# bridgedp/hunter_bipedal_control

Measured on AMD Instinct MI355X. Metric: MPC+WBC updates/sec (batch=4096, N=100, 12-DoF), higher is better.
Workload: dtype f64; 1 GPU; 4096 distinct hunter instances (4096/GPU, state seed 1234 + id), trot gait from t = 0.1, cmd_vel (0.3, 0, 0, 0), N=100 shooting intervals (dt 0.015 s), node tables generated on the device (hb_refgen_update, per-knot IK joint references), 1 SQP iteration + WeightedWbc per update, x0 of every call perturbed by measurement noise (sigma 0.01) so that no call re-solves a converged problem: every line s; batch_per_gpu=4096, total_instances=4096, horizon_nodes=100

## Files before the change

hunter_bipedal_control_amd/csrc/hb_lq.hpp:

```cpp
#pragma once
#include "hb_model.hpp"
#include "hb_tile.hpp"

namespace hb {

struct DevConfig {
  double Q_diag[HB_NX];
  double R_FF_diag[12];
  double R_jj[HB_NJ * HB_NJ];
  double friction_mu, friction_reg, friction_gripper, friction_shift, fb_mu, fb_delta;
  double soft_w;
  double pos_b[2], vel_b[2], force_b[2], force_lim[2];
  double kp_normal, zv_gain, zv_off, xy_gain;
  double g_max, g_min, alpha_decay, alpha_min, gamma_c, armijo, delta_tol;
  double torque_limits[5];
  double wbc_mu, swing_kp, swing_kd, bh_kp, bh_kd, ba_kp, ba_kd, w_swing, w_base, w_force, wbc_eps;
  int wbc_max_iter, wbc_type;
  double default_joint_state[HB_NJ];
  int debug_stop;
  int wbc_reg_steps;
  int wbc_eps_mode;
};

constexpr int NU_T = 12;
constexpr int REC_LD = 36, REC_CV = 22, REC_CU = 23;
constexpr int REC_AB = 0;
constexpr int REC_PR = 792;
constexpr int REC_QT = 1224;
constexpr int REC_QT_PACKED = 254;
constexpr int REC_qT = REC_QT + REC_QT_PACKED;
HB_HD constexpr int rec_Qidx(int i, int c) { return (i * (43 - i)) / 2 + c; }
constexpr int REC_RICCATI_END = 1730;
constexpr int REC_KX = 1730;
constexpr int REC_KE = 1950;
constexpr int REC_Z = 1960;
constexpr int REC_DF = 2020;
constexpr int REC_QF = 2032;
constexpr int REC_RF = 2054;
constexpr int REC_META = 2076;
constexpr int REC_DT = REC_META + 6;
constexpr int REC_DQ = REC_META + 8;
constexpr int REC_RX_END = REC_DQ + 10;
constexpr int REC_SIZE = 2112;
constexpr int GAIN_SIZE = 288;
HB_HD constexpr int rec_A(int i, int c) { return REC_AB + i * REC_LD + c; }
HB_HD constexpr int rec_B(int i, int a) { return REC_AB + i * REC_LD + REC_CU + a; }
HB_HD constexpr int rec_b(int i) { return REC_AB + i * REC_LD + REC_CV; }
HB_HD constexpr int rec_P(int a, int c) { return REC_PR + a * REC_LD + c; }
HB_HD constexpr int rec_R(int a, int c) { return REC_PR + a * REC_LD + REC_CU + c; }
HB_HD constexpr int rec_r(int a) { return REC_PR + a * REC_LD + REC_CV; }
inline void rec_unpack(const double* rec, double* A, double* B, double* b, double* Q, double* P, double* R, double* q, double* r, int* n_til) {
  for (int i = 0; i < 22; ++i) {
    for (int c = 0; c < 22; ++c) {
      if (A) A[i * 22 + c] = rec[rec_A(i, c)];
      if (Q) Q[i * 22 + c] = rec[REC_QT + (i <= c ? rec_Qidx(i, c) : rec_Qidx(c, i))];
    }
    for (int a = 0; a < NU_T; ++a)
      if (B) B[i * NU_T + a] = rec[rec_B(i, a)];
    if (b) b[i] = rec[rec_b(i)];
    if (q) q[i] = rec[REC_qT + i];
  }
  for (int a = 0; a < NU_T; ++a) {
    for (int c = 0; c < 22; ++c)
      if (P) P[a * 22 + c] = rec[rec_P(a, c)];
    for (int c = 0; c < NU_T; ++c)
      if (R) R[a * NU_T + c] = rec[rec_R(a, c)];
    if (r) r[a] = rec[rec_r(a)];
  }
  if (n_til) *n_til = int(rec[REC_META]) + int(rec[REC_META + 1]);
}
HB_HD void rec_unpack_recovery(const double* rec, double* Kx, double* ke, double* Z, double* dF, double* qf, double* rf, double* meta,
                               double* dt, double* dq) {
  const auto copy = [rec](double* dst, int at, int n) {
    if (dst)
      for (int i = 0; i < n; ++i) dst[i] = rec[at + i];
  };
  copy(Kx, REC_KX, 220); copy(ke, REC_KE, 10); copy(Z, REC_Z, 60); copy(dF, REC_DF, 12); copy(qf, REC_QF, 22); copy(rf, REC_RF, 22);
  copy(meta, REC_META, 6); copy(dt, REC_DT, 1); copy(dq, REC_DQ, 10);
}

struct RelaxedBarrierD {
  double mu, delta;
  HB_HD double value(double h) const {
    if (h > delta) return -mu * log_t(h);
    const double z = (h - 2.0 * delta) * rcp_t(delta);
    return mu * (-log_t(delta) + 0.5 * z * z - 0.5);
  }
  HB_HD double d1(double h) const { const double r = rcp_t(h > delta ? h : delta); return h > delta ? -mu * r : mu * (h - 2.0 * delta) * r * r; }
  HB_HD double d2(double h) const { const double r = rcp_t(h > delta ? h : delta); return mu * r * r; }
};

struct LqLds {
  static constexpr int CDt = 0;
  static constexpr int rowval = CDt + 384;
  static constexpr int xs = rowval + 12;
  static constexpr int us = xs + 22;
  static constexpr int fv = us + 22;
  static constexpr int scal = fv;
  static constexpr int xe = fv + 24;
  static constexpr int xplus = xe;
  static constexpr int ABt = xe + 22;
  static constexpr int W = ABt + 528;
  static constexpr int Pj = W;
  static constexpr int LDK = 29;
  static constexpr int Kx = W + 230;
  static constexpr int Z = Kx + 23;
  static constexpr int GtG = Kx + 124;
  static constexpr int btmp = fv;
  static constexpr int ints = Kx + 10 * LDK;
  static constexpr int park = ints + 16;
  static constexpr int xnext_park = fv;
  static constexpr int tail_end = park + 22;
  static constexpr int Mm = ABt;
  static constexpr int RFF = Mm + 10 * LDK;
  static constexpr int qx = RFF + 36;
  static constexpr int ru = qx + 22;
  static constexpr int Qd = ru + 22;
  static constexpr int Rjj = Qd + 22;
  static constexpr int LJ = ABt;
#if defined(__HIP_DEVICE_COMPILE__)
  static constexpr int J1 = ABt + 528;
#else
  static constexpr int J1 = LJ + 4 * LEGJ_SIZE;
#endif
  static constexpr int J2 = J1 + 29 * 9;
  static constexpr int LVP = 27;
  static constexpr int LV = J2 + 29 * 9;
#if defined(__HIP_DEVICE_COMPILE__)
  static constexpr int p1_end = LV + 2 * LVP;
  static constexpr int SC = fv + 12;
  HB_HD static constexpr int fr_slot(int pt, int i) { return LV + pt * LVP + 15 + 6 * (i & 1) + 3 * (i >> 1); }
#else
  static constexpr int FRh = LV + 2 * LVP;
  static constexpr int SC = FRh + 24;
  static constexpr int p1_end = SC + 12;
  HB_HD static constexpr int fr_slot(int pt, int i) { return FRh + 12 * pt + 3 * i; }
#endif
  static constexpr int total = p1_end > tail_end ? p1_end : tail_end;
};
static_assert(LqLds::J1 >= LqLds::ABt + 528, "ABt is written while J1 / J2 are still being read");
static_assert(LqLds::park >= LqLds::J1, "the parked states are written behind the compose: they lie over J1 / J2 / the leg values, which it has finished with by then");
static_assert(LqLds::Rjj + 100 <= LqLds::ABt + 528, "M | R_FF | q_x | r_u | Q-diagonal | R_jj must fit over ABt");
#if defined(__HIP_DEVICE_COMPILE__)
static_assert(LqLds::total * 8 <= 12800, "k_lq: LDS per node must allow 12 workgroups per CU (10 allocation granules of 1280 B, DESIGN.md 3.1)");
#endif
HB_HD int cd_row(int dir) { return dir < 22 ? dir : dir - 12; }
HB_HD int j_row(int dir) { return dir < 6 ? dir : (dir < 22 ? dir - 3 : dir - 15); }
HB_HD int j_dir(int row) { return row < 6 ? row : (row < 19 ? row + 3 : row + 15); }
HB_HD int j_col(int frow) { return frow < 6 ? frow - 3 : (frow < 9 ? frow : frow - 6); }
HB_HD int j_frow(int col) { return col < 3 ? col + 3 : (col < 6 ? col + 6 : col); }
HB_HD int c_slot(int i, int a) { return a == 0 ? 8 + i : 4 * (i & 1) + 2 * (i >> 1) + (a - 1); }
HB_HD int slot_foot(int s) { return s < 8 ? (s >> 2) + 2 * ((s >> 1) & 1) : s - 8; }
HB_HD bool slot_normal(int s) { return s >= 8; }
HB_HD bool slot_is_eq(int s, int cfm) { return slot_normal(s) || ((cfm >> slot_foot(s)) & 1); }
HB_HD bool slot_is_soft(int s, int cfm) { return !slot_normal(s) && !((cfm >> slot_foot(s)) & 1); }
struct EqStepLive { int cfm; HB_HD bool operator()(int j) const { return j == 2 || ((cfm >> j) & 5) != 0; } };
struct SoftStepLive { int cfm; HB_HD bool operator()(int j) const { return j != 2 && ((~cfm >> j) & 5) != 0; } };

HB_HD LegLayout lq_leg_layout() { LegLayout l; l.compact = true; l.pair_sum = true; return l; }

struct NodeIn {
  const double* x;
  const double* u;
  const double* xnext;
  const double* xref;
  const double* swing;
  double dt;
  int mode;
  bool preloaded = false;
  double x_lane = 0.0, u_lane = 0.0;
  const LegJointConst* jc = nullptr;
  bool consts = false;
  double c_tab = 0.0;
};

struct LqP1 {
  double *xs, *us, *xe, *fv, *LV_all, *SC, *J1, *J2, *CDt, *rowval, *LJ_all;
};
HB_HD LqP1 lq_p1(double* lds) {
  LqP1 p;
  p.xs = lds + LqLds::xs;
  p.us = lds + LqLds::us;
  p.xe = lds + LqLds::xe;
  p.fv = lds + LqLds::fv;
  p.LV_all = lds + LqLds::LV;
  p.SC = lds + LqLds::SC;
  p.J1 = lds + LqLds::J1;
  p.J2 = lds + LqLds::J2;
  p.CDt = lds + LqLds::CDt;
  p.rowval = lds + LqLds::rowval;
  p.LJ_all = lds + LqLds::LJ;
  return p;
}

HB_HD int lq_ms_slot(int pt, int e) { return (2 * pt + e / 5) * LEGJ_SIZE + (e % 5) * LEGJ_STRIDE + LEGJ_MS; }
constexpr int LQ_CV_IINV = 0, LQ_CV_WB = 6, LQ_CV_LJ = 9, LQ_CV_P = 12;
struct LqPointValues {
  Vec3<double> fr[HB_NC], fvel[HB_NC];
  Mat3<double> R;
  Vec3<double> wb, P, hb, lj, omega, euler_rate, v_lin, com_rel;
  Sym3<double> Iinv;
  double icy;
};
HB_HD void lq_point_values(const DevModel& M, const double* LV, const double* zyx_sc , const double* hn, LqPointValues& o) {
  const double mb = M.mass[0], mt = M.total_mass;
  const Vec3<double> cb(M.com[0][0], M.com[0][1], M.com[0][2]);
  Sym3<double> Ib;
  Ib.xx = M.inertia[0][0]; Ib.xy = M.inertia[0][1]; Ib.xz = M.inertia[0][2];
  Ib.yy = M.inertia[0][3]; Ib.yz = M.inertia[0][4]; Ib.zz = M.inertia[0][5];
  const Vec3<double> mc = ld3(LV + 0) + mb * cb;
  const Sym3<double> IO = ld6(LV + 3) + Ib + point_inertia<double>(mb, cb);
  o.lj = ld3(LV + 9);
  const Vec3<double> LjO = ld3(LV + 12);
  const double inv_m = rcp_t(mt);
  o.P = inv_m * mc;
  Sym3<double> Ic = IO;
  {
    const Sym3<double> sh = point_inertia<double>(mt, o.P);
    Ic.xx -= sh.xx; Ic.xy -= sh.xy; Ic.xz -= sh.xz; Ic.yy -= sh.yy; Ic.yz -= sh.yz; Ic.zz -= sh.zz;
  }
  {
    const double c00 = Ic.yy * Ic.zz - Ic.yz * Ic.yz, c01 = Ic.xz * Ic.yz - Ic.xy * Ic.zz, c02 = Ic.xy * Ic.yz - Ic.xz * Ic.yy;
    const double c11 = Ic.xx * Ic.zz - Ic.xz * Ic.xz, c12 = Ic.xy * Ic.xz - Ic.xx * Ic.yz, c22 = Ic.xx * Ic.yy - Ic.xy * Ic.xy;
    const double inv = rcp_t(Ic.xx * c00 + Ic.xy * c01 + Ic.xz * c02);
    o.Iinv.xx = inv * c00; o.Iinv.xy = inv * c01; o.Iinv.xz = inv * c02; o.Iinv.yy = inv * c11; o.Iinv.yz = inv * c12; o.Iinv.zz = inv * c22;
  }
  const double sz = zyx_sc[0], cz = zyx_sc[1], sy = zyx_sc[2], cy = zyx_sc[3], sx = zyx_sc[4], cx = zyx_sc[5];
  Mat3<double>& R = o.R;
  R.m[0] = cz * cy; R.m[1] = cz * sy * sx - sz * cx; R.m[2] = cz * sy * cx + sz * sx;
  R.m[3] = sz * cy; R.m[4] = sz * sy * sx + cz * cx; R.m[5] = sz * sy * cx - cz * sx;
  R.m[6] = -sy;     R.m[7] = cy * sx;                R.m[8] = cy * cx;
  o.icy = rcp_t(cy);
  o.hb = tmul(R, Vec3<double>(mt * hn[3], mt * hn[4], mt * hn[5]));
  const Vec3<double> Lj = LjO - cross(o.P, o.lj);
  o.wb = o.Iinv * (o.hb - Lj);
  o.omega = R * o.wb;
  {
    const double roll_rate = (cz * o.omega.x + sz * o.omega.y) * o.icy;
    o.euler_rate = Vec3<double>(o.omega.z + sy * roll_rate, cz * o.omega.y - sz * o.omega.x, roll_rate);
  }
  o.com_rel = R * o.P;
  o.v_lin = Vec3<double>(hn[0], hn[1], hn[2]) - cross(o.omega, o.com_rel) - inv_m * (R * o.lj);
// ... 253 lines not shown
    W[k * 23 + 22] = s;
  }
  cx.sync();
  double* Lc = Kx;
  double* col = Kx + 100;
  double* Linv = Kx + 112;
  int rank_l = 0, donemask = 0;
  int ei0 = 0, ej0 = cx.lane;
  while (ej0 > ei0) { ej0 -= ei0 + 1; ++ei0; }
#if defined(__HIP_DEVICE_COMPILE__)
  {
    static_assert(Ctx::nlanes == 64, "one triangle element per lane");
    const bool own = cx.lane < 55;
    const bool diag = own && ei0 == ej0;
    double g = own ? GtG[ei0 * 10 + ej0] : 0.0;
    const double tol = 1e-10 * wave_max_pos_f64(diag ? g : 0.0);
    for (int i = cx.lane; i < 124; i += cx.nlanes) Kx[i] = 0.0;
    cx.sync();
    for (int st = 0; st < 10; ++st) {
      const double v = (diag && !((donemask >> ei0) & 1)) ? g : -1.0;
      const double best = wave_max_pos_f64(v);
      if (!(best > tol)) break;
      const unsigned long long hit = __ballot(v == best);
      const int ps = __builtin_amdgcn_readlane(ei0, __ffsll(hit) - 1);
      const double rinv = rsqrt_t(best), lss = best * rinv;
      if (own && (ei0 == ps || ej0 == ps)) {
        const int k = (ei0 == ps) ? ej0 : ei0;
        if (!((donemask >> k) & 1)) {
          const double l = (k == ps) ? lss : g * rinv;
          col[k] = l;
          Lc[st * 10 + k] = l;
        }
      }
      if (cx.lane == 0) { perm[st] = ps; Linv[st] = rinv; }
      cx.sync();
      donemask |= 1 << ps;
      if (own && !((donemask >> ei0) & 1) && !((donemask >> ej0) & 1)) g -= col[ei0] * col[ej0];
      cx.sync();
      rank_l = st + 1;
    }
  }
#else
  double tol;
  {
    double dmax0 = 0;
    for (int i = 0; i < 10; ++i) dmax0 = fmax(dmax0, GtG[i * 10 + i]);
    tol = 1e-10 * dmax0;
  }
  for (int i = cx.lane; i < 124; i += cx.nlanes) Kx[i] = 0.0;
  cx.sync();
  for (int st = 0; st < 10; ++st) {
    int ps = -1;
    double best = -1.0;
    for (int i = 0; i < 10; ++i) {
      const double dv = GtG[i * 11];
      if (!((donemask >> i) & 1) && dv > best) { best = dv; ps = i; }
    }
    if (!(best > tol)) break;
    const double rinv = rsqrt_t(best), lss = best * rinv;
    for (int k = cx.lane; k < 10; k += cx.nlanes) {
      if (!((donemask >> k) & 1)) {
        const double l = (k == ps) ? lss : GtG[(k > ps ? k * 10 + ps : ps * 10 + k)] * rinv;
        col[k] = l;
        Lc[st * 10 + k] = l;
      }
    }
    if (cx.lane == 0) { perm[st] = ps; Linv[st] = rinv; }
    cx.sync();
    donemask |= 1 << ps;
    for (int e = cx.lane; e < 55; e += cx.nlanes) {
      int i = ei0, j = ej0;
      if (e != cx.lane) { i = 0; j = e; while (j > i) { j -= i + 1; ++i; } }
      if (!((donemask >> i) & 1) && !((donemask >> j) & 1)) GtG[i * 10 + j] -= col[i] * col[j];
    }
    cx.sync();
    rank_l = st + 1;
  }
#endif
  if (cx.lane == 0) {
    int w = rank_l;
    for (int i = 0; i < 10; ++i)
      if (!((donemask >> i) & 1)) perm[w++] = i;
  }
  cx.sync();
  HB_ABLATE_STOP(C.debug_stop == form::LQ_FACTOR);
  const int rank = rank_l;
  const int nz = 10 - rank;
  {
    double Lr[45], dinv[10];
    int pm[10];
#pragma unroll
    for (int a = 0; a < 10; ++a) { pm[a] = perm[a]; dinv[a] = Linv[a]; }
#pragma unroll
    for (int a = 1; a < 10; ++a) {
#pragma unroll
      for (int t = 0; t < a; ++t) Lr[a * (a - 1) / 2 + t] = Lc[t * 10 + pm[a]];
    }
    cx.sync();
    auto write_col = [Kx, Z, &pm, rank](int c, bool zlive, int pf, const double* y) {
      if (c < 23) {
#pragma unroll
        for (int a = 0; a < 10; ++a) Kx[pm[a] * LqLds::LDK + c] = y[a];
      } else {
#pragma unroll
        for (int a = 0; a < 10; ++a) Z[pm[a] * LqLds::LDK + c - 23] = zlive ? (a < rank ? -y[a] : (pm[a] == pf ? 1.0 : 0.0)) : 0.0;
      }
    };
#if !defined(__HIP_DEVICE_COMPILE__)
    double ycols[29][10];
    bool ylive[29];
    int ypf[29];
#endif
    for (int cc = cx.lane; cc < 29; cc += cx.nlanes) {
      const int c = 28 - cc;
      const bool isz = c >= 23;
      const int bz = c - 23;
      const bool zlive = isz && bz < nz;
      const int pf = zlive ? perm[rank + bz] : 0;
      double y[10];
#pragma unroll
      for (int a = 0; a < 10; ++a) {
        double sacc = -W[pm[a] * 23 + (isz ? 0 : c)];
#pragma unroll
        for (int t = 0; t < a; ++t) sacc -= Lr[a * (a - 1) / 2 + t] * y[t];
        y[a] = sacc * dinv[a];
      }
      if (isz) {
#pragma unroll
        for (int a = 0; a < 10; ++a) y[a] = zlive ? Lc[a * 10 + pf] : 0.0;
      }
#pragma unroll
      for (int a = 9; a >= 0; --a) {
        double sacc = y[a];
#pragma unroll
        for (int t = a + 1; t < 10; ++t) sacc -= Lr[t * (t - 1) / 2 + a] * y[t];
        y[a] = sacc * dinv[a];
      }
#if defined(__HIP_DEVICE_COMPILE__)
      write_col(c, zlive, pf, y);
#else
      for (int a = 0; a < 10; ++a) ycols[c][a] = y[a];
      ylive[c] = zlive;
      ypf[c] = pf;
#endif
    }
#if !defined(__HIP_DEVICE_COMPILE__)
    cx.sync();
    for (int cc = cx.lane; cc < 29; cc += cx.nlanes) write_col(cc, ylive[cc], ypf[cc], ycols[cc]);
#endif
  }

  HB_ABLATE_STOP(C.debug_stop == form::LQ_SOLVES);
#if defined(__HIP_DEVICE_COMPILE__)
  double cw_reg = 0.0, clo_reg = 0.0, chi_reg = 0.0;
  double rj0_reg = 0.0, rj1_reg = 0.0;
  if (in.consts) {
    rj0_reg = C.R_jj[cx.lane];
    if (cx.lane < 36) rj1_reg = C.R_jj[64 + cx.lane];
    __builtin_amdgcn_sched_barrier(0);
  }
  if (!in.consts) {
    const int role = cx.lane;
    if (role < 22) {
      cw_reg = C.Q_diag[role];
      if (role >= 12) { clo_reg = M.q_lower[role - 12]; chi_reg = M.q_upper[role - 12]; }
    } else if (role < 34) {
      cw_reg = C.R_FF_diag[role - 22];
    } else if (role < 44) {
      clo_reg = M.qd_limit[role - 34];
    }
  }
#endif
  for (int i = cx.lane; i < 22; i += cx.nlanes) xplus[i] -= xnext_at(i);
  cx.sync();
  const int ntil = n_f + nz;
  int flist = 0;
  {
    int cnt = 0;
    for (int i = 0; i < HB_NC; ++i)
      if (cf[i]) { flist |= i << (2 * cnt); ++cnt; }
  }
  double* btmp = lds + LqLds::btmp;
  {
    WaveTile<1, 2> ta;
    tile_init(cx, ta, 12, 22, [ABt](int row, int c) { return ABt[c * 12 + row]; });
    tile_mma<12, 12, true, LDK, false, 10>(cx, ta, ABt + 34 * 12, Kx, 12, LDK);
#if defined(__HIP_DEVICE_COMPILE__)
    if (in.consts) {
      W[cx.lane] = rj0_reg;
      if (cx.lane < 36) W[64 + cx.lane] = rj1_reg;
      __builtin_amdgcn_sched_barrier(0);
    }
#endif
    tile_store_rm_cols<REC_LD>(cx, ta, 12, 0, 22, rec + rec_A(0, 0));
    tile_store_rm_cols<1>(cx, ta, 12, 22, 23, btmp - 22);
    tile_store_rm_cols<REC_LD>(cx, ta, 12, 23, 23 + nz, rec + rec_A(0, 0) + n_f);
  }
  for (int c = cx.lane; c < 22; c += cx.nlanes) {
#pragma unroll
    for (int j = 0; j < 10; ++j) {
      const double kx = Kx[j * LDK + c];
      rec[rec_A(12 + j, c)] = (c == 12 + j ? 1.0 : 0.0) + dt * kx;
      rec[REC_KX + j * 22 + c] = kx;
    }
  }
  cx.sync();
  HB_ABLATE_STOP(C.debug_stop == form::LQ_DEFECT);
  for (int row = cx.lane; row < 22; row += cx.nlanes) {
#pragma unroll
    for (int col = 0; col < NU_T; ++col) {
      if (col < n_f) {
        const int foot = (flist >> (2 * (col / 3))) & 3;
        rec[rec_B(row, col)] = row < 12 ? ABt[(22 + 3 * foot + col % 3) * 12 + row] : 0.0;
      } else if (col >= ntil) {
        rec[rec_B(row, col)] = 0.0;
      } else if (row >= 12) {
        rec[rec_B(row, col)] = dt * Z[(row - 12) * LDK + col - n_f];
      }
    }
    double s = xplus[row];
    if (row >= 12) rec[REC_DQ + row - 12] = s;
    if (row < 12) {
      s += btmp[row];
      for (int i = 0; i < HB_NC; ++i)
        if (!cf[i])
          for (int a = 0; a < 3; ++a) s -= ABt[(22 + 3 * i + a) * 12 + row] * us[3 * i + a];
    } else {
      s += dt * Kx[(row - 12) * LDK + 22];
    }
    rec[rec_b(row)] = s;
  }
  HB_ABLATE_STOP(C.debug_stop == form::LQ_B_COLUMNS);
  double* red = Mm;
  {
    int nc = 0;
    for (int i = 0; i < HB_NC; ++i) nc += cf[i];
    const double fz_nom = nc > 0 ? M.total_mass * M.gravity / nc : 0.0;
    const RelaxedBarrierD fb{C.fb_mu, C.fb_delta};
    const RelaxedBarrierD bp{C.pos_b[0], C.pos_b[1]}, bv{C.vel_b[0], C.vel_b[1]}, bf{C.force_b[0], C.force_b[1]};
    auto cone = [&](int i, double& h, double* g, double& H00, double& H01, double& H11) {
      const double Fx = us[3 * i], Fy = us[3 * i + 1], Fz = us[3 * i + 2];
      const double t2 = Fx * Fx + Fy * Fy + C.friction_reg, tn = sqrt(t2), t32 = tn * t2;
      h = C.friction_mu * (Fz + C.friction_gripper) - tn;
      const double itn = rcp_t(tn), it32 = rcp_t(t32);
      g[0] = -Fx * itn; g[1] = -Fy * itn; g[2] = C.friction_mu;
      H00 = -(Fy * Fy + C.friction_reg) * it32; H01 = Fx * Fy * it32; H11 = -(Fx * Fx + C.friction_reg) * it32;
    };
    double* coneb = Rjj;
    for (int i = cx.lane; i < HB_NC; i += cx.nlanes) {
      double h = 1.0, g[3] = {0.0, 0.0, 0.0}, H00 = 0.0, H01 = 0.0, H11 = 0.0, pv = 0.0, p1 = 0.0, p2 = 0.0;
      if (cf[i]) {
        cone(i, h, g, H00, H01, H11);
        pv = fb.value(h); p1 = fb.d1(h); p2 = fb.d2(h);
      }
      double* cb = coneb + 12 * i;
      cb[0] = h; cb[1] = g[0]; cb[2] = g[1]; cb[3] = g[2]; cb[4] = H00; cb[5] = H01; cb[6] = H11; cb[7] = pv; cb[8] = p1; cb[9] = p2;
    }
    cx.sync();
    double shift_sum = 0;
    for (int i = 0; i < HB_NC; ++i)
      if (cf[i]) shift_sum += -coneb[12 * i + 8] * C.friction_shift;
#if defined(__HIP_DEVICE_COMPILE__)
    double rff_reg[3] = {0.0, 0.0, 0.0};
    const double* Rc_lds = C.R_jj;
    if (in.consts) {
      const int l = cx.lane, foot = (l - 56) & 3;
      const double g1 = wave_gather_f64(in.c_tab, l < 22 ? l + 22 : (l < 44 ? l + 20 : 22 + 3 * foot));
      const double g2 = wave_gather_f64(in.c_tab, l < 22 ? l + 32 : 23 + 3 * foot);
      const double g3 = wave_gather_f64(in.c_tab, 24 + 3 * foot);
      cw_reg = in.c_tab;
      clo_reg = g1;
      chi_reg = g2;
      rff_reg[0] = g1; rff_reg[1] = g2; rff_reg[2] = g3;
      Rc_lds = W;
    }
#endif
    for (int role = cx.lane; role < 64; role += cx.nlanes) {
      double pc = 0, pd = 0, pe = 0;
      double bval = 0.0, bd1 = 0.0, bd2 = 0.0;
      {
        bool hasb = false;
        double h1 = 1.0, h2 = 1.0, bmu = 0.0, bdel = 1.0;
        if (role >= 12 && role < 22) {
          const int j = role - 12;
          const double h = xs[role];
#if defined(__HIP_DEVICE_COMPILE__)
          (void)j;
          hasb = true; h1 = h - clo_reg; h2 = chi_reg - h; bmu = bp.mu; bdel = bp.delta;
#else
          hasb = true; h1 = h - M.q_lower[j]; h2 = M.q_upper[j] - h; bmu = bp.mu; bdel = bp.delta;
#endif
        } else if (role >= 22 && role < 34) {
          const int m = role - 22;
          if (m - 3 * (m / 3) == 2) {
            const double h = us[m];
            hasb = true; h1 = h - C.force_lim[0]; h2 = C.force_lim[1] - h; bmu = bf.mu; bdel = bf.delta;
          }
        } else if (role >= 34 && role < 44) {
          const int k = role - 34;
#if defined(__HIP_DEVICE_COMPILE__)
          const double hv = us[12 + k], vl = clo_reg;
#else
          const double hv = us[12 + k], vl = M.qd_limit[k];
#endif
          hasb = true; h1 = hv + vl; h2 = vl - hv; bmu = bv.mu; bdel = bv.delta;
        }
        if (hasb) {
          const RelaxedBarrierD rb{bmu, bdel};
          bval = rb.value(h1) + rb.value(h2);
          bd1 = rb.d1(h1) - rb.d1(h2);
          bd2 = rb.d2(h1) + rb.d2(h2);
        }
      }
      if (role < 22) {
        const int i = role;
        const double dxv = xs[i] - xref_at(i);
#if defined(__HIP_DEVICE_COMPILE__)
        const double Qi = cw_reg;
#else
        const double Qi = C.Q_diag[i];
#endif
        double qd_ = Qi + shift_sum, qg = Qi * dxv;
        pc += 0.5 * Qi * dxv * dxv;
        if (i >= 12) {
          pc += bval;
          qg += bd1;
          qd_ += bd2;
        }
        Qd[i] = qd_;
        qx[i] = qg;
        const double dd = xplus[i];
        pd += dd * dd;
      } else if (role < 34) {
        const int m = role - 22, foot = m / 3, a = m % 3;
        const double du = us[m] - ((a == 2 && cf[foot]) ? fz_nom : 0.0);
#if defined(__HIP_DEVICE_COMPILE__)
        const double Rm_ = cw_reg;
#else
        const double Rm_ = C.R_FF_diag[m];
#endif
        double rg = Rm_ * du;
        pc += 0.5 * Rm_ * du * du;
        if (cf[foot]) {
          rg += coneb[12 * foot + 8] * coneb[12 * foot + 1 + a];
        } else {
          pe += us[m] * us[m];
        }
        if (a == 2) {
          pc += bval;
          rg += bd1;
        }
        ru[m] = rg;
      } else if (role < 44) {
        const int k = role - 34;
        double sacc = 0;
#if defined(__HIP_DEVICE_COMPILE__)
        for (int l = 0; l < HB_NJ; ++l) sacc += Rc_lds[k * 10 + l] * us[12 + l];
#else
        for (int l = 0; l < HB_NJ; ++l) sacc += C.R_jj[k * 10 + l] * us[12 + l];
#endif
        pc += 0.5 * us[12 + k] * sacc;
        pc += bval;
        ru[12 + k] = sacc + bd1;
        scal[4 + k] = bd2 + shift_sum;
      } else if (role < 56) {
        const int sl = role - 44;
        const double rv = rowval[sl];
        if (slot_is_eq(sl, cfm)) pe += rv * rv;
        else pc += 0.5 * C.soft_w * rv * rv;
      } else if (role < 60) {
        const int foot = role - 56;
        double blk[9];
        for (int e = 0; e < 9; ++e) blk[e] = 0.0;
#if defined(__HIP_DEVICE_COMPILE__)
        for (int a = 0; a < 3; ++a) blk[4 * a] = (in.consts ? rff_reg[a] : C.R_FF_diag[3 * foot + a]) + shift_sum;
#else
        for (int a = 0; a < 3; ++a) blk[4 * a] = C.R_FF_diag[3 * foot + a] + shift_sum;
#endif
        {
          const double h = us[3 * foot + 2];
          blk[8] += bf.d2(h - C.force_lim[0]) + bf.d2(C.force_lim[1] - h);
        }
        if (cf[foot]) {
          const double* cb = coneb + 12 * foot;
          const double g[3] = {cb[1], cb[2], cb[3]}, H00 = cb[4], H01 = cb[5], H11 = cb[6];
          const double p1 = cb[8], p2 = cb[9];
          pc += cb[7];
          for (int a = 0; a < 3; ++a)
            for (int bb = 0; bb < 3; ++bb) blk[3 * a + bb] += p2 * g[a] * g[bb];
          blk[0] += p1 * H00; blk[1] += p1 * H01; blk[3] += p1 * H01; blk[4] += p1 * H11;
        }
        for (int e = 0; e < 9; ++e) RFF[9 * foot + e] = blk[e];
      }
#if defined(__HIP_DEVICE_COMPILE__)
      pc = wave_sum_f64(pc);
      pd = wave_sum_f64(pd);
      pe = wave_sum_f64(pe);
      if (role == 0) { scal[0] = pc; scal[1] = pd; scal[2] = pe; }
#else
      red[role] = pc;
      red[64 + role] = pd;
      red[128 + role] = pe;
#endif
    }
  }
  cx.sync();
#if !defined(__HIP_DEVICE_COMPILE__)
  for (int w = cx.lane; w < 3; w += cx.nlanes) {
    double sacc = 0;
    for (int l = 0; l < 64; ++l) sacc += red[64 * w + l];
    scal[w] = sacc;
  }
  cx.sync();
#endif
  HB_ABLATE_STOP(C.debug_stop == form::LQ_COST);
  for (int c = cx.lane; c < 32; c += cx.nlanes) {
    double s = 0;
#pragma unroll
    for (int slot = 0; slot < 8; ++slot) {
      const double w = slot_is_soft(slot, cfm) ? 1.0 : 0.0;
      s += (w * rowval[slot]) * CDt[c * 12 + slot];
    }
    if (c < 22) qx[c] += C.soft_w * s;
    else ru[12 + c - 22] += C.soft_w * s;
  }
  {
    const double sw = C.soft_w;
#if defined(__HIP_DEVICE_COMPILE__)
    const double* Rc = in.consts ? W : C.R_jj;
#else
    const double* Rc = C.R_jj;
#endif
    WaveTile<1, 2> tg;
    tile_init(cx, tg, 10, 32, [Rc, scal](int k, int r) {
      const int rr = (r >= 22 ? r : 22) - 22;
      const double v = Rc[k * 10 + rr], sc = scal[4 + k];
      return r >= 22 ? v + (rr == k ? sc : 0.0) : 0.0;
    });
    tile_mma<12, 12, false, 12, true>(cx, tg, CDt + 22 * 12, CDt, 10, 32, [cfm, sw](int slot) { return slot_is_soft(slot, cfm) ? sw : 0.0; },
                                      SoftStepLive{cfm});
    tile_store(cx, tg, 10, 32, [Pj, Rjj](int k, int r, double v) {
      double* dst = r < 22 ? Pj + k * 22 + r : Rjj + k * 10 + r - 22;
      *dst = v;
    });
  }
  cx.sync();
  {
    WaveTile<1, 2> tm;
    tile_init(cx, tm, 10, 23, [Pj, ru](int k, int c) {
      const double a = Pj[k * 22 + (c < 22 ? c : 21)], b = ru[12 + k];
      return c < 22 ? a : b;
    });
    tile_mma<12, 10, false, LDK, false, 10>(cx, tm, Rjj, Kx, 10, LDK);
    tile_store_rm<LDK>(cx, tm, 10, LDK, Mm);
  }
  cx.sync();

  HB_ABLATE_STOP(C.debug_stop == form::LQ_SOFT_ROWS);
  {
    const double sw = C.soft_w;
    auto soft = [cfm, sw](int slot) { return slot_is_soft(slot, cfm) ? sw : 0.0; };
    const SoftStepLive soft_live{cfm};
    WaveTile<1, 2> t0;
    WaveTile<1, 1> t1;
    tile_init(cx, t0, 16, 22, [Qd](int a, int b) { const double d = Qd[a]; return a == b ? d : 0.0; });
    tile_init(cx, t1, 6, 6, [Qd](int a, int b) { const double d = Qd[16 + a]; return a == b ? d : 0.0; });
    tile_mma<12, 12, false, 12, true>(cx, t0, CDt, CDt, 16, 22, soft, soft_live);
    tile_mma<12, 12, false, 12, true>(cx, t1, CDt + 16 * 12, CDt + 16 * 12, 6, 6, soft, soft_live);
    tile_set_col(cx, t0, 22, 16, [qx](int a) { return qx[a]; });
    tile_set_col(cx, t1, 6, 6, [qx](int a) { return qx[16 + a]; });
    tile_mma<12, LDK, true, LDK, false, 10>(cx, t0, Kx, Mm, 16, 23);
    tile_mma<12, LDK, true, LDK, false, 10>(cx, t1, Kx + 16, Mm + 16, 6, 7);
    tile_mma<12, 22, true, LDK, false, 10>(cx, t0, Pj, Kx, 16, 23);
    tile_mma<12, 22, true, LDK, false, 10>(cx, t1, Pj + 16, Kx + 16, 6, 7);
    tile_store(cx, t0, 16, 23, [rec, dt](int a, int b, double v) {
      double* dst = b < 22 ? rec + REC_QT + rec_Qidx(a, b) : rec + REC_qT + a;
      if (a <= b) *dst = dt * v;
    });
    tile_store(cx, t1, 6, 7, [rec, dt](int a, int b, double v) {
      double* dst = b < 6 ? rec + REC_QT + rec_Qidx(16 + a, 16 + b) : rec + REC_qT + 16 + a;
      if (a <= b) *dst = dt * v;
    });
  }
  HB_ABLATE_STOP(C.debug_stop == form::LQ_Q);
  for (int a = cx.lane; a < 22; a += cx.nlanes) {
    rec[REC_QF + a] = dt * qx[a];
    rec[REC_RF + a] = dt * ru[a];
  }
  if (nz > 0) {
    WaveTile<1, 2> tp;
    tile_init(cx, tp, 6, 22, [](int, int) { return 0.0; });
    tile_mma<12, LDK, true, LDK, false, 10>(cx, tp, Z, Mm, 6, LDK);
    tile_store_rm_cols<REC_LD>(cx, tp, nz, 0, 23, rec + rec_P(n_f, 0), dt);
    tile_store_rm_cols<REC_LD>(cx, tp, nz, 23, 23 + nz, rec + rec_P(n_f, 0) + n_f, dt);
  }
  for (int c = cx.lane; c < 22; c += cx.nlanes) {
#pragma unroll
    for (int a = 0; a < NU_T; ++a)
      if (a < n_f || a >= ntil) rec[rec_P(a, c)] = 0.0;
  }
  HB_ABLATE_STOP(C.debug_stop == form::LQ_P);
  for (int idx = cx.lane; idx < NU_T * NU_T; idx += cx.nlanes) {
    const int ca = idx / NU_T, cb = idx % NU_T;
    double s = 0.0;
    bool pad_diag = false;
    if (ca < n_f && cb < n_f) {
      if (ca / 3 == cb / 3) {
        const int foot = (flist >> (2 * (ca / 3))) & 3;
        s = RFF[9 * foot + 3 * (ca % 3) + (cb % 3)];
      }
    } else if (ca >= n_f && ca < ntil && cb >= n_f && cb < ntil) {
      continue;
    } else if (ca >= ntil && ca == cb) {
      pad_diag = true;
    }
    rec[rec_R(ca, cb)] = pad_diag ? 1.0 : dt * s;
  }
  for (int col = cx.lane; col < NU_T; col += cx.nlanes) {
    double s = 0.0;
    if (col < n_f) {
      const int foot = (flist >> (2 * (col / 3))) & 3;
      s = ru[3 * foot + col % 3];
    } else if (col < ntil) {
      continue;
    }
    rec[rec_r(col)] = dt * s;
  }
  HB_ABLATE_STOP(C.debug_stop == form::LQ_R);
  for (int k = cx.lane; k < 10; k += cx.nlanes) rec[REC_KE + k] = Kx[k * LDK + 22];
  for (int idx = cx.lane; idx < 60; idx += cx.nlanes) rec[REC_Z + idx] = idx % 6 < nz ? Z[(idx / 6) * LDK + idx % 6] : 0.0;
  for (int i = cx.lane; i < 12; i += cx.nlanes) rec[REC_DF + i] = cf[i / 3] ? 0.0 : -us[i];
  if (cx.lane == 0) {
    rec[REC_META + 0] = double(n_f);
    rec[REC_META + 1] = double(nz);
    rec[REC_META + 2] = double(in.mode);
// ... 476 lines not shown
```

Before: 544,300 updates/s.

## Evaluate every relaxed barrier once per lane and combine pairs via wave gathers

```diff
diff --git a/hunter_bipedal_control_amd/csrc/hb_lq.hpp b/hunter_bipedal_control_amd/csrc/hb_lq.hpp
--- a/hunter_bipedal_control_amd/csrc/hb_lq.hpp
+++ b/hunter_bipedal_control_amd/csrc/hb_lq.hpp
@@ -88,6 +88,18 @@
   }
   HB_HD double d1(double h) const { const double r = rcp_t(h > delta ? h : delta); return h > delta ? -mu * r : mu * (h - 2.0 * delta) * r * r; }
   HB_HD double d2(double h) const { const double r = rcp_t(h > delta ? h : delta); return mu * r * r; }
+  HB_HD void eval(double h, double& v, double& p1, double& p2, double& r, double& f1, double& f2) const {
+    const bool lg = h > delta;
+    const double a = lg ? h : delta;
+    const double L = log_t(a);
+    r = rcp_t(a);
+    const double z = (h - 2.0 * delta) * r;
+    v = lg ? -mu * L : mu * (-L + 0.5 * z * z - 0.5);
+    f1 = lg ? -mu : mu * (h - 2.0 * delta) * r;
+    f2 = mu * r;
+    p1 = f1 * r;
+    p2 = f2 * r;
+  }
 };
 
 struct LqLds {
@@ -647,7 +659,7 @@
 
   HB_ABLATE_STOP(C.debug_stop == form::LQ_SOLVES);
 #if defined(__HIP_DEVICE_COMPILE__)
-  double cw_reg = 0.0, clo_reg = 0.0, chi_reg = 0.0;
+  double cw_reg = 0.0, clo_reg = 0.0;
   double rj0_reg = 0.0, rj1_reg = 0.0;
   if (in.consts) {
     rj0_reg = C.R_jj[cx.lane];
@@ -655,15 +667,13 @@
     __builtin_amdgcn_sched_barrier(0);
   }
   if (!in.consts) {
-    const int role = cx.lane;
-    if (role < 22) {
-      cw_reg = C.Q_diag[role];
-      if (role >= 12) { clo_reg = M.q_lower[role - 12]; chi_reg = M.q_upper[role - 12]; }
-    } else if (role < 34) {
-      cw_reg = C.R_FF_diag[role - 22];
-    } else if (role < 44) {
-      clo_reg = M.qd_limit[role - 34];
-    }
+    const int l = cx.lane;
+    if (l < 22) cw_reg = C.Q_diag[l];
+    else if (l < 34) cw_reg = C.R_FF_diag[l - 22];
+    if (l >= 2 && l < 12) clo_reg = M.qd_limit[l - 2];
+    else if (l >= 12 && l < 22) clo_reg = M.q_lower[l - 12];
+    else if (l >= 34 && l < 44) clo_reg = M.qd_limit[l - 34];
+    else if (l >= 44 && l < 54) clo_reg = M.q_upper[l - 44];
   }
 #endif
   for (int i = cx.lane; i < 22; i += cx.nlanes) xplus[i] -= xnext_at(i);
@@ -735,13 +745,76 @@
     const RelaxedBarrierD bp{C.pos_b[0], C.pos_b[1]}, bv{C.vel_b[0], C.vel_b[1]}, bf{C.force_b[0], C.force_b[1]};
     auto cone = [&](int i, double& h, double* g, double& H00, double& H01, double& H11) {
       const double Fx = us[3 * i], Fy = us[3 * i + 1], Fz = us[3 * i + 2];
+#if defined(__HIP_DEVICE_COMPILE__)
+      double fxx = Fx * Fx, fyy = Fy * Fy;
+      asm("" : "+v"(fxx), "+v"(fyy));
+      const double t2 = fma(Fx, Fx, fyy) + C.friction_reg, tn = sqrt(t2), t32 = tn * t2;
+      h = fma(C.friction_mu, Fz + C.friction_gripper, -tn);
+      const double itn = rcp_t(tn), it32 = rcp_t(t32);
+      g[0] = -Fx * itn; g[1] = -Fy * itn; g[2] = C.friction_mu;
+      H00 = -(fyy + C.friction_reg) * it32; H01 = Fx * Fy * it32; H11 = -(fxx + C.friction_reg) * it32;
+#else
       const double t2 = Fx * Fx + Fy * Fy + C.friction_reg, tn = sqrt(t2), t32 = tn * t2;
       h = C.friction_mu * (Fz + C.friction_gripper) - tn;
       const double itn = rcp_t(tn), it32 = rcp_t(t32);
       g[0] = -Fx * itn; g[1] = -Fy * itn; g[2] = C.friction_mu;
       H00 = -(Fy * Fy + C.friction_reg) * it32; H01 = Fx * Fy * it32; H11 = -(Fx * Fx + C.friction_reg) * it32;
+#endif
     };
     double* coneb = Rjj;
+#if defined(__HIP_DEVICE_COMPILE__)
+    static_assert(Ctx::nlanes == 64, "one barrier argument per lane");
+    static_assert(LqLds::us == LqLds::xs + 22, "(x, u) is one array of 44 for the barrier pass");
+    int bl = cx.lane;
+    if (!in.consts) asm volatile("" : "+v"(bl));
+    const int bfoot = bl & 3;
+    double rff_reg[3] = {0.0, 0.0, 0.0};
+    const double* Rc_lds = C.R_jj;
+    if (in.consts) {
+      const double g1 = wave_gather_f64(in.c_tab, bl < 12 ? bl + 52 : (bl < 22 ? bl + 22 : (bl < 44 ? bl + 20 : (bl < 54 ? bl : 22 + 3 * bfoot))));
+      const double g2 = wave_gather_f64(in.c_tab, 23 + 3 * bfoot);
+      const double g3 = wave_gather_f64(in.c_tab, 24 + 3 * bfoot);
+      cw_reg = in.c_tab;
+      clo_reg = g1;
+      rff_reg[0] = g1; rff_reg[1] = g2; rff_reg[2] = g3;
+      Rc_lds = W;
+    }
+    double bval, bd1, bd2;
+    {
+      const int l32 = bl & 31;
+      const bool is_pos = unsigned(l32 - 12) < 10u, is_vel = unsigned(l32 - 2) < 10u;
+      const bool is_flo = bl >= 24 && bl < 34 && (bl - 22) % 3 == 2, is_fhi = bl >= 56 && bl < 60;
+      const bool is_cone = bl >= 60 && cf[bfoot];
+      const bool upper = bl < 12 || bl >= 44;
+      const double y = (lds + LqLds::xs)[bl < 12 ? bl + 32 : (bl < 44 ? bl : (bl < 54 ? bl - 32 : 24 + 3 * bfoot))];
+      const double lim = is_flo ? C.force_lim[0] : (is_fhi ? C.force_lim[1] : clo_reg);
+      const double h_lo = (is_vel ? y + lim : y - lim), h_hi = lim - y;
+      const bool hasb = is_pos || is_vel || is_flo || is_fhi || is_cone;
+      double h = (is_pos || is_vel || is_flo || is_fhi) ? (upper ? h_hi : h_lo) : 1.0;
+      double* cb = coneb + 12 * bfoot;
+      if (bl >= 60) {
+        double cg[3] = {0.0, 0.0, 0.0}, H00 = 0.0, H01 = 0.0, H11 = 0.0;
+        if (is_cone) cone(bfoot, h, cg, H00, H01, H11);
+        cb[0] = h; cb[1] = cg[0]; cb[2] = cg[1]; cb[3] = cg[2]; cb[4] = H00; cb[5] = H01; cb[6] = H11;
+      }
+      const double bmu = (is_pos ? bp.mu : (is_vel ? bv.mu : ((is_flo || is_fhi) ? bf.mu : (is_cone ? fb.mu : 0.0))));
+      const double bdel = (is_pos ? bp.delta : (is_vel ? bv.delta : ((is_flo || is_fhi) ? bf.delta : (is_cone ? fb.delta : 1.0))));
+      double pv, p1, p2, br, f1, f2;
+      RelaxedBarrierD{bmu, bdel}.eval(h, pv, p1, p2, br, f1, f2);
+      pv = hasb ? pv : 0.0; p1 = hasb ? p1 : 0.0; p2 = hasb ? p2 : 0.0;
+      if (bl >= 60) { cb[7] = pv; cb[8] = p1; cb[9] = p2; }
+      const int src = (is_pos || is_vel) ? (bl ^ 32) : (is_flo ? 56 + (((bl - 24) * 11) >> 5) : (is_fhi ? 24 + 3 * bfoot : bl));
+      bval = pv + wave_gather_f64(pv, src);
+      bd1 = fma(f1, br, -wave_gather_f64(p1, src));
+      bd2 = fma(f2, br, wave_gather_f64(p2, src));
+      const double bd2_role = wave_gather_f64(bd2, src);
+      bd2 = is_fhi ? bd2_role : bd2;
+    }
+    cx.sync();
+    double shift_sum = 0;
+    for (int i = 0; i < HB_NC; ++i)
+      if (cf[i]) shift_sum += -coneb[12 * i + 8] * C.friction_shift;
+#else
     for (int i = cx.lane; i < HB_NC; i += cx.nlanes) {
       double h = 1.0, g[3] = {0.0, 0.0, 0.0}, H00 = 0.0, H01 = 0.0, H11 = 0.0, pv = 0.0, p1 = 0.0, p2 = 0.0;
       if (cf[i]) {
@@ -755,23 +828,10 @@
     double shift_sum = 0;
     for (int i = 0; i < HB_NC; ++i)
       if (cf[i]) shift_sum += -coneb[12 * i + 8] * C.friction_shift;
-#if defined(__HIP_DEVICE_COMPILE__)
-    double rff_reg[3] = {0.0, 0.0, 0.0};
-    const double* Rc_lds = C.R_jj;
-    if (in.consts) {
-      const int l = cx.lane, foot = (l - 56) & 3;
-      const double g1 = wave_gather_f64(in.c_tab, l < 22 ? l + 22 : (l < 44 ? l + 20 : 22 + 3 * foot));
-      const double g2 = wave_gather_f64(in.c_tab, l < 22 ? l + 32 : 23 + 3 * foot);
-      const double g3 = wave_gather_f64(in.c_tab, 24 + 3 * foot);
-      cw_reg = in.c_tab;
-      clo_reg = g1;
-      chi_reg = g2;
-      rff_reg[0] = g1; rff_reg[1] = g2; rff_reg[2] = g3;
-      Rc_lds = W;
-    }
 #endif
     for (int role = cx.lane; role < 64; role += cx.nlanes) {
       double pc = 0, pd = 0, pe = 0;
+#if !defined(__HIP_DEVICE_COMPILE__)
       double bval = 0.0, bd1 = 0.0, bd2 = 0.0;
       {
         bool hasb = false;
@@ -779,12 +839,7 @@
         if (role >= 12 && role < 22) {
           const int j = role - 12;
           const double h = xs[role];
-#if defined(__HIP_DEVICE_COMPILE__)
-          (void)j;
-          hasb = true; h1 = h - clo_reg; h2 = chi_reg - h; bmu = bp.mu; bdel = bp.delta;
-#else
           hasb = true; h1 = h - M.q_lower[j]; h2 = M.q_upper[j] - h; bmu = bp.mu; bdel = bp.delta;
-#endif
         } else if (role >= 22 && role < 34) {
           const int m = role - 22;
           if (m - 3 * (m / 3) == 2) {
@@ -793,11 +848,7 @@
           }
         } else if (role >= 34 && role < 44) {
           const int k = role - 34;
-#if defined(__HIP_DEVICE_COMPILE__)
-          const double hv = us[12 + k], vl = clo_reg;
-#else
           const double hv = us[12 + k], vl = M.qd_limit[k];
-#endif
           hasb = true; h1 = hv + vl; h2 = vl - hv; bmu = bv.mu; bdel = bv.delta;
         }
         if (hasb) {
@@ -807,6 +858,7 @@
           bd2 = rb.d2(h1) + rb.d2(h2);
         }
       }
+#endif
       if (role < 22) {
         const int i = role;
         const double dxv = xs[i] - xref_at(i);
@@ -872,10 +924,14 @@
 #else
         for (int a = 0; a < 3; ++a) blk[4 * a] = C.R_FF_diag[3 * foot + a] + shift_sum;
 #endif
+#if defined(__HIP_DEVICE_COMPILE__)
+        blk[8] += bd2;
+#else
         {
           const double h = us[3 * foot + 2];
           blk[8] += bf.d2(h - C.force_lim[0]) + bf.d2(C.force_lim[1] - h);
         }
+#endif
         if (cf[foot]) {
           const double* cb = coneb + 12 * foot;
           const double g[3] = {cb[1], cb[2], cb[3]}, H00 = cb[4], H01 = cb[5], H11 = cb[6];
```

After: 548,400 updates/s, median of 6. No clear change (+0.7%).
